# ChunLI-666/PointCloudProcessor

Hardware: AMD Instinct MI355X
Metric: Mpoints×frames/sec colorized (higher is better)
Workload: dtype f32/f64

## Files before the change

include/pcp_hip.h:

```cpp
#ifndef PCP_HIP_H
#define PCP_HIP_H

#include <stdint.h>

#ifdef __cplusplus
extern "C" {
#endif

#define PCP_ABI_VERSION 6

#define PCP_OK 0
#define PCP_ERR_INVALID (-1)
#define PCP_ERR_STATE (-2)
#define PCP_ERR_DEVICE (-3)
#define PCP_ERR_NOMEM (-4)
#define PCP_ERR_RANGE (-5)

typedef struct pcp_context pcp_context;

typedef struct pcp_pose {
  double x, y, z, qw, qx, qy, qz;
} pcp_pose;

typedef struct pcp_camera {
// ... 168 lines not shown
int pcp_nid_accumulate(pcp_context *ctx, const double T[16], int32_t bins);
int pcp_nid_histograms_device(pcp_context *ctx, void **device_ptr, int64_t *count);
int pcp_nid_finish(pcp_context *ctx, int32_t bins, double *cost, double grad6[6], int32_t *valid);
typedef int (*pcp_nid_eval_fn)(void *user, const double T[16], int32_t bins, double *cost, double grad6[6], int32_t *valid);
int pcp_nid_optimize_with(pcp_context *ctx, pcp_nid_eval_fn eval, void *user, const double T_init[16], int32_t bins,
                          int32_t max_outer_iterations, double T_out[16], double *final_cost, int32_t *evaluations);

int pcp_close_pairs(pcp_context *ctx, double radius, int64_t *points_with_close_neighbour);

int pcp_timing_enable(pcp_context *ctx, int32_t on);
int pcp_timing_reset(pcp_context *ctx);
int pcp_timing_get(pcp_context *ctx, int32_t kernel_id, double *total_ms, int64_t *launches);
const char *pcp_kernel_name(int32_t kernel_id);
int pcp_tile_mask_density(pcp_context *ctx, double *kept_fraction);
int pcp_tile_masks(pcp_context *ctx, int64_t *tiles, int32_t *mask_words, uint32_t *out_words);
int pcp_sor_redo_fraction(pcp_context *ctx, double *fraction);
int pcp_sor_distances(pcp_context *ctx, int64_t capacity, float *out_distance);
int pcp_selftest_arithmetic(pcp_context *ctx, int64_t samples, uint64_t seed, int64_t *mismatches_fp64,
                            int64_t *mismatches_fp32);

#ifdef __cplusplus
}
#endif
#endif
```

pointcloudprocessor_amd/capi.py:

```python
from __future__ import annotations

import ctypes as C
import os
import re

import numpy as np

from . import _build

PCP_OK = 0
PCP_ERR_INVALID = -1
PCP_ERR_STATE = -2
PCP_ERR_DEVICE = -3
PCP_ERR_NOMEM = -4
PCP_ERR_RANGE = -5

NID_EVAL_FN = C.CFUNCTYPE(C.c_int, C.c_void_p, C.POINTER(C.c_double), C.c_int32, C.POINTER(C.c_double), C.POINTER(C.c_double),
                          C.POINTER(C.c_int32))
K_PROJECT, K_DEPTH, K_COLOUR, K_VISIBILITY, K_MLS_GRID, K_MLS_FIT, K_MISC, K_SOR, K_MLS_VOXEL, K_TILE_MASK, K_NID, K_HPR = range(12)
K_COLOUR_SMOOTH = 12
K_COUNT = 13


class PcpError(RuntimeError):
# ... 627 lines not shown
        self._check(self.lib.pcp_tile_mask_density(self.h, C.byref(v)))
        return v.value

    def selftest_arithmetic(self, samples: int = 1 << 26, seed: int = 1):
        a, b = C.c_int64(), C.c_int64()
        self._check(self.lib.pcp_selftest_arithmetic(self.h, C.c_int64(samples), C.c_uint64(seed), C.byref(a), C.byref(b)))
        return a.value, b.value

    def tile_masks(self) -> np.ndarray:
        t, w = C.c_int64(), C.c_int32()
        self._check(self.lib.pcp_tile_masks(self.h, C.byref(t), C.byref(w), None))
        out = np.empty((t.value, w.value), np.uint32)
        self._check(self.lib.pcp_tile_masks(self.h, None, None, _ptr(out)))
        return out

    def kernel_name(self, kernel_id: int) -> str:
        return self.lib.pcp_kernel_name(C.c_int32(kernel_id)).decode()
```

pointcloudprocessor_amd/csrc/pcp_colour.hip:

```cpp
#include <algorithm>
#include <cfloat>
#include <cstdlib>

#include "pcp_device.hpp"
#include "pcp_hsv.hpp"
#include "pcp_scan.hpp"

namespace pcp {

constexpr int kBlock = 256;
constexpr uint32_t kFltMaxBits = 0x7f7fffffu;

template <bool kCommon>
__device__ __forceinline__ DevCamera common_camera(const DevCamera &in) {
  DevCamera c = in;
  if constexpr (kCommon) {
    c.cull_mode = PCP_CULL_ZBUFFER;
    c.enable_zbuf = 1;
    c.pretest = 1;
    c.ds_fast = 1;
  }
  return c;
}
inline bool is_common_camera(const DevCamera &c) {
// ... 127 lines not shown
  Interval rc = iv_add(iv_add(iv_scale(c.k1, r2), iv_scale(c.k2, r4)), iv_scale(c.k3, r6));
  rc.lo += 1.0;
  rc.hi += 1.0;
  const Interval t1 = iv_scale(2.0, iv_mul(xn, yn));
  const Interval t2 = iv_add(r2, iv_scale(2.0, x2));
  const Interval t3 = iv_add(r2, iv_scale(2.0, y2));
  const Interval xd = iv_pad(iv_add(iv_add(iv_mul(rc, xn), iv_scale(c.p1, t1)), iv_scale(c.p2, t2)));
  const Interval yd = iv_pad(iv_add(iv_add(iv_mul(rc, yn), iv_scale(c.p1, t3)), iv_scale(c.p2, t1)));
  Interval u = iv_pad(iv_scale(c.fx, xd)), v = iv_pad(iv_scale(c.fy, yd));
  u.lo += c.cx; u.hi += c.cx;
  v.lo += c.cy; v.hi += c.cy;
  if (!isfinite(u.lo + u.hi + v.lo + v.hi)) return 0;
  if (u.hi < static_cast<double>(c.u_lo) || u.lo > static_cast<double>(c.u_hi) ||
      v.hi < static_cast<double>(c.v_lo) || v.lo > static_cast<double>(c.v_hi))
    return 1;
  return (u.lo > static_cast<double>(c.u_lo) + 1.0 && u.hi < static_cast<double>(c.u_hi) - 1.0 &&
          v.lo > static_cast<double>(c.v_lo) + 1.0 && v.hi < static_cast<double>(c.v_hi) - 1.0)
             ? 2
             : 0;
}

constexpr int kTileGroup = 16;

__global__ __launch_bounds__(kBlock) void k_group_mask_flat(const float4 *__restrict__ spheres, int64_t groups, DevCamera cam,
                                                            const DevFrame *__restrict__ frames, int32_t n_frames,
                                                            int32_t w0, int32_t w1, int32_t words,
                                                            uint32_t *__restrict__ group_mask,
                                                            uint32_t *__restrict__ group_inside, int32_t cull_enabled,
                                                            int32_t *__restrict__ zeroed, int32_t n_zeroed,
                                                            unsigned long long *__restrict__ far_maps, int64_t far_cells) {
  const int64_t idx = static_cast<int64_t>(blockIdx.x) * kBlock + threadIdx.x;
  if (idx < n_zeroed) zeroed[idx] = 0;
// ... 157 lines not shown

__device__ __forceinline__ uint32_t range_bits(int32_t w, int32_t f0, int32_t f1) {
  const int32_t fb = max(f0, w << 5), fe = min(f1, (w << 5) + 32);
  const int32_t nb = fe - fb;
  return nb <= 0 ? 0u : (((nb >= 32) ? 0xffffffffu : ((1u << nb) - 1u)) << (fb & 31));
}

template <bool kCommon>
__global__ __launch_bounds__(kBlock) void k_depth_pass(const float *__restrict__ x, const float *__restrict__ y,
                                                       const float *__restrict__ z, int64_t n, DevCamera cam_in,
                                                       const DevFrame *__restrict__ frames, int32_t f0, int32_t f1,
                                                       unsigned long long *__restrict__ depth, int64_t cells,
                                                       int32_t depth_first_frame, uint32_t *__restrict__ tile_mask,
                                                       const uint32_t *__restrict__ tile_inside, int32_t words,
                                                       const int32_t *__restrict__ tile_order) {
  DevCamera cam = common_camera<kCommon>(cam_in);
  if constexpr (kCommon) cam.pretest = 0;
  __shared__ unsigned long long combine[kBlock];
  const int lane = threadIdx.x & 63;
  unsigned long long *tbl = combine + (threadIdx.x & ~63);
  const int64_t j = tile_order ? static_cast<int64_t>(tile_order[blockIdx.x]) * 64 + threadIdx.x
                               : static_cast<int64_t>(xcd_chunked_block()) * kBlock + threadIdx.x;
  const bool live = j < n;
  if (!__ballot(live)) return;
  const float px = live ? x[j] : 0.0f, py = live ? y[j] : 0.0f, pz = live ? z[j] : 0.0f;
  const int64_t tile = __builtin_amdgcn_readfirstlane(static_cast<int32_t>(j >> 6));
  const bool finite_sure = cam.frames_bounded != 0 && __all(fabsf(px) <= 0x1p40f && fabsf(py) <= 0x1p40f && fabsf(pz) <= 0x1p40f);
  unsigned long long *held_at = nullptr;
  unsigned long long held_bits = 0ull, held_seen = 0ull;
  auto settle_held = [&]() {
    if (held_at && held_bits < held_seen) atomicMin(held_at, held_bits);
    held_at = nullptr;
  };
  for (int32_t w = f0 >> 5; w <= (f1 - 1) >> 5; ++w) {
    const uint32_t in_range = range_bits(w, f0, f1);
    uint32_t todo = in_range;
    if (tile_mask) todo &= tile_mask[tile * words + w];
    todo = __builtin_amdgcn_readfirstlane(todo);
    const uint32_t inside = tile_inside ? __builtin_amdgcn_readfirstlane(tile_inside[tile * words + w]) : 0u;
    uint32_t seen = 0u;
    while (todo) {
      const int32_t b = __builtin_ctz(todo);
      const int32_t f = (w << 5) + b;
      todo &= todo - 1u;
      const DevFrame &fr = frames[f];
      const Projected p = project_point(cam, fr.w2c, px, py, pz, ((inside >> b) & 1u) == 0u, finite_sure);
      const bool in_map = live && p.cell >= 0;
      const bool cand = live && p.pixel >= 0 && (cam.enable_zbuf ? p.cell >= 0 : p.cell != -1);
      if (__ballot(cand)) seen |= 1u << b;
      settle_held();
      if (cam.enable_zbuf && __ballot(in_map)) {
        unsigned long long *map = depth + static_cast<uint64_t>(static_cast<uint32_t>(f - depth_first_frame)) * static_cast<uint32_t>(cells);
        unsigned long long key = ~0ull, sbits = 0ull;
        if (in_map) {
          sbits = static_cast<unsigned long long>(__double_as_longlong(sumsq64(p.xc, p.yc, p.zc)));
          key = (static_cast<unsigned long long>(static_cast<uint32_t>(p.cell)) << 32) | (sbits >> 32);
        }
        tbl[lane] = ~0ull;
        __builtin_amdgcn_wave_barrier();
        if (in_map) atomicMin(&tbl[p.cell & 63], key);
        __builtin_amdgcn_wave_barrier();
        if (in_map) {
          const unsigned long long got = tbl[p.cell & 63];
          if (got == key || static_cast<uint32_t>(got >> 32) != static_cast<uint32_t>(p.cell)) {
// ... 39 lines not shown
  float *score;
  uint32_t *rgb;
  int32_t *frame;
  int32_t *count;
};

struct MatchArgs {
  const uint8_t *in_a;
  unsigned long long *moved;
  float e2;
};

struct LabelOut {
  uint32_t *word;
};

template <bool kCommon, int kMatch, bool kOneShot, bool kLabel = false>
__global__ __launch_bounds__(kBlock) void k_colour_pass(const float *__restrict__ x, const float *__restrict__ y,
                                                        const float *__restrict__ z, int64_t n, DevCamera cam_in,
                                                        const DevFrame *__restrict__ frames, int32_t f0, int32_t f1,
                                                        const uint32_t *__restrict__ depth, int64_t cells,
                                                        const uint32_t *__restrict__ tile_mask, int32_t words,
                                                        const uint32_t *__restrict__ images, int64_t image_px,
                                                        TopState st, const int32_t *__restrict__ perm,
                                                        uint32_t *__restrict__ rgba, int32_t flags_in,
                                                        const uint32_t *__restrict__ hull_bits_in, MatchArgs mb,
                                                        [[maybe_unused]] LabelOut lab) {
  DevCamera cam = common_camera<kCommon>(cam_in);
  if constexpr (kMatch == 1) cam.match_mode = PCP_MATCH_IDENTITY;
  if constexpr (kMatch == 2 || kMatch == 3) cam.match_mode = PCP_MATCH_ROUNDTRIP;
  const uint32_t *__restrict__ hull_bits = kCommon ? nullptr : hull_bits_in;
  const int32_t flags = kOneShot ? 4 : flags_in;
  const int64_t j = static_cast<int64_t>(xcd_chunked_block()) * kBlock + threadIdx.x;
  const bool live = j < n;
  if (!__ballot(live)) return;
  const float px = live ? x[j] : 0.0f, py = live ? y[j] : 0.0f, pz = live ? z[j] : 0.0f;
  const int64_t tile = __builtin_amdgcn_readfirstlane(static_cast<int32_t>(j >> 6));
  const bool finite_sure = cam.frames_bounded != 0 && __all(fabsf(px) <= 0x1p40f && fabsf(py) <= 0x1p40f && fabsf(pz) <= 0x1p40f);
  Top5 t;
  t.init();
  if ((flags & 1) && live) {
    t.s0 = st.score[0 * n + j]; t.s1 = st.score[1 * n + j]; t.s2 = st.score[2 * n + j];
    t.s3 = st.score[3 * n + j]; t.s4 = st.score[4 * n + j];
    t.c0 = st.rgb[0 * n + j]; t.c1 = st.rgb[1 * n + j]; t.c2 = st.rgb[2 * n + j];
    t.c3 = st.rgb[3 * n + j]; t.c4 = st.rgb[4 * n + j];
    t.f0 = st.frame[0 * n + j]; t.f1 = st.frame[1 * n + j]; t.f2 = st.frame[2 * n + j];
    t.f3 = st.frame[3 * n + j]; t.f4 = st.frame[4 * n + j];
    t.count = st.count[j];
  }
  [[maybe_unused]] bool in_a = false;
  [[maybe_unused]] uint32_t moved = 0u;
  if constexpr (kMatch == 3) in_a = live && mb.in_a[j] != 0;
  for (int32_t w = f0 >> 5; w <= (f1 - 1) >> 5; ++w) {
    uint32_t todo = range_bits(w, f0, f1);
    if (tile_mask) todo &= tile_mask[tile * words + w];
    todo = __builtin_amdgcn_readfirstlane(todo);
    const uint32_t hull_word = (hull_bits && live) ? hull_bits[static_cast<int64_t>(w) * n + j] : 0xffffffffu;
    while (todo) {
      const int32_t f = (w << 5) + __builtin_ctz(todo);
      todo &= todo - 1u;
      const DevFrame &fr = frames[f];
      const Projected p = project_point<false>(cam, fr.w2c, px, py, pz, true, finite_sure);
      const bool cand = live && p.pixel >= 0 && (cam.enable_zbuf ? p.cell >= 0 : p.cell != -1) &&
                        ((hull_word >> (f & 31)) & 1u);
// ... 6 lines not shown
          if (keep) keep = roundtrip_sample_moved(cam, fr, px, py, pz, sx, sy, sz, mb.e2, moved) && !in_a;
        } else {
          if (cam.match_mode == PCP_MATCH_ROUNDTRIP && keep) keep = roundtrip_sample(cam, fr, px, py, pz, sx, sy, sz);
        }
        if (keep) {
          const uint32_t texel = images[static_cast<uint64_t>(static_cast<uint32_t>(f)) * static_cast<uint32_t>(image_px) + static_cast<uint32_t>(p.pixel)];
          t.insert(final_score(sx, sy, sz, fr.px, fr.py, fr.pz), kLabel ? texel : texel & 0xffffffu, f);
        }
      }
    }
  }
  if constexpr (kMatch == 3) {
    if (moved) atomicAdd(mb.moved, static_cast<unsigned long long>(moved));
  }
  if (!live) return;
  if (flags & 2) {
    st.score[0 * n + j] = t.s0; st.score[1 * n + j] = t.s1; st.score[2 * n + j] = t.s2;
    st.score[3 * n + j] = t.s3; st.score[4 * n + j] = t.s4;
    st.rgb[0 * n + j] = t.c0; st.rgb[1 * n + j] = t.c1; st.rgb[2 * n + j] = t.c2;
    st.rgb[3 * n + j] = t.c3; st.rgb[4 * n + j] = t.c4;
    st.frame[0 * n + j] = t.f0; st.frame[1 * n + j] = t.f1; st.frame[2 * n + j] = t.f2;
    st.frame[3 * n + j] = t.f3; st.frame[4 * n + j] = t.f4;
    st.count[j] = t.count;
  }
  if (flags & 4) {
    const int64_t o = perm[j];
    rgba[o] = t.finalise();
    if constexpr (kLabel) {
      uint32_t bad = 0u;
      lab.word[o] = t.labels(bad);
      if (bad) lab.word[n] = 1u;
    }
  }
}

__device__ __forceinline__ Top5 load_top5(const TopState &st, int64_t n, int64_t j) {
  Top5 t;
  t.s0 = st.score[0 * n + j]; t.s1 = st.score[1 * n + j]; t.s2 = st.score[2 * n + j];
  t.s3 = st.score[3 * n + j]; t.s4 = st.score[4 * n + j];
  t.c0 = st.rgb[0 * n + j]; t.c1 = st.rgb[1 * n + j]; t.c2 = st.rgb[2 * n + j];
  t.c3 = st.rgb[3 * n + j]; t.c4 = st.rgb[4 * n + j];
  t.f0 = st.frame[0 * n + j]; t.f1 = st.frame[1 * n + j]; t.f2 = st.frame[2 * n + j];
  t.f3 = st.frame[3 * n + j]; t.f4 = st.frame[4 * n + j];
  t.count = st.count[j];
  return t;
}
__global__ __launch_bounds__(kBlock) void k_finalise(int64_t n, TopState st, const int32_t *__restrict__ perm,
                                                     uint32_t *__restrict__ rgba) {
  const int64_t j = static_cast<int64_t>(blockIdx.x) * kBlock + threadIdx.x;
  if (j >= n) return;
  const Top5 t = load_top5(st, n, j);
  rgba[static_cast<int64_t>(perm[j])] = t.finalise();
}
__global__ __launch_bounds__(kBlock) void k_finalise_labels(int64_t n, TopState st, const int32_t *__restrict__ perm,
                                                            uint32_t *__restrict__ rgba, LabelOut lab) {
  const int64_t j = static_cast<int64_t>(blockIdx.x) * kBlock + threadIdx.x;
  if (j >= n) return;
  const Top5 t = load_top5(st, n, j);
  const int64_t o = perm[j];
  rgba[o] = t.finalise();
  uint32_t bad = 0u;
  lab.word[o] = t.labels(bad);
  if (bad) lab.word[n] = 1u;
}

template <bool kLabel>
__global__ __launch_bounds__(kBlock) void k_match_fixup(const float *__restrict__ x, const float *__restrict__ y,
                                                        const float *__restrict__ z, int64_t n, DevCamera cam,
                                                        const DevFrame *__restrict__ frames, int32_t f0, int32_t f1,
                                                        const uint32_t *__restrict__ depth, int64_t cells,
                                                        const uint32_t *__restrict__ tile_mask, int32_t words,
                                                        const uint32_t *__restrict__ images, int64_t image_px, TopState st,
                                                        const int32_t *__restrict__ perm, uint32_t *__restrict__ rgba,
                                                        int32_t flags, const uint32_t *__restrict__ hull_bits,
                                                        const int32_t *__restrict__ list, int64_t na,
                                                        const int64_t *__restrict__ off, const int32_t *__restrict__ cols,
                                                        [[maybe_unused]] LabelOut lab) {
  const int64_t a = static_cast<int64_t>(blockIdx.x) * kBlock + threadIdx.x;
// ... 55 lines not shown
}

template <bool kLabel>
inline auto colour_pass_kernel(bool common, int32_t match_mode, int32_t flags) {
  auto kernel = k_colour_pass<false, 0, false, kLabel>;
  if (common && match_mode == PCP_MATCH_IDENTITY)
    kernel = flags == 4 ? k_colour_pass<true, 1, true, kLabel> : k_colour_pass<true, 1, false, kLabel>;
  if (common && match_mode == PCP_MATCH_ROUNDTRIP)
    kernel = flags == 4 ? k_colour_pass<true, 2, true, kLabel> : k_colour_pass<true, 2, false, kLabel>;
  if (match_mode == PCP_MATCH_RADIUS)
    kernel = !common ? k_colour_pass<false, 3, false, kLabel>
                     : flags == 4 ? k_colour_pass<true, 3, true, kLabel> : k_colour_pass<true, 3, false, kLabel>;
  return kernel;
}

__device__ __forceinline__ uint64_t mix64(uint64_t v) {
  v += 0x9e3779b97f4a7c15ull;
  v = (v ^ (v >> 30)) * 0xbf58476d1ce4e5b9ull;
  v = (v ^ (v >> 27)) * 0x94d049bb133111ebull;
  return v ^ (v >> 31);
}
__device__ __forceinline__ bool same_f64(double a, double b) {
  if (a != a && b != b) return true;
  if (a == 0.0 && b == 0.0) return true;
  return __double_as_longlong(a) == __double_as_longlong(b);
}

__global__ __launch_bounds__(kBlock) void k_selftest_div64(int64_t samples, uint64_t seed,
                                                           unsigned long long *__restrict__ bad) {
  const int64_t i = static_cast<int64_t>(blockIdx.x) * kBlock + threadIdx.x;
// ... 328 lines not shown
                     ctx->mask_words, ctx->tile_work.p, ctx->work_hist.p);
  hipLaunchKernelGGL(k_work_scatter, dim3(sort_blocks), dim3(kBlock), 0, ctx->stream, ctx->tile_work.p, ctx->n_tiles,
                     ctx->work_hist.p, ctx->work_hist.p + kWorkBins, order);
  PCP_HIP_TRY(ctx, hipGetLastError());
  return PCP_OK;
}

static int ensure_hull_bits(pcp_context *ctx) {
  const size_t words = static_cast<size_t>((ctx->n_frames + 31) / 32);
  const size_t need = words * static_cast<size_t>(ctx->n) + 4;
  if (ctx->hull_bits.count < need || ctx->hull_valid.size() != static_cast<size_t>(ctx->n_frames)) {
    PCP_HIP_TRY(ctx, ctx->hull_bits.ensure(need));
    ctx->hull_valid.assign(static_cast<size_t>(ctx->n_frames), 0);
  }
  return PCP_OK;
}

static int ensure_depth(pcp_context *ctx) {
  const size_t need = static_cast<size_t>(cells_of(ctx)) * ctx->n_frames + 4;
  if (ctx->depth.count < need) {
    PCP_HIP_TRY(ctx, ctx->depth.ensure(need));
    std::fill(ctx->depth_valid.begin(), ctx->depth_valid.end(), uint8_t(0));
  }
  const int32_t words = (ctx->n_frames + 31) / 32;
  const size_t need_mask = static_cast<size_t>(words) * static_cast<size_t>(std::max<int64_t>(ctx->n_tiles, 1)) + 4;
  if (ctx->tile_mask.count < need_mask || ctx->mask_words != words) {
    PCP_HIP_TRY(ctx, ctx->tile_mask.ensure(need_mask));
    PCP_HIP_TRY(ctx, ctx->tile_inside.ensure(need_mask));
    PCP_HIP_TRY(ctx, ctx->tile_work.ensure(static_cast<size_t>(std::max<int64_t>(ctx->n_tiles, 1)) + 4));
    PCP_HIP_TRY(ctx, ctx->tile_order.ensure(static_cast<size_t>(std::max<int64_t>(ctx->n_tiles, 1)) + 4));
// ... 551 lines not shown
    return set_error(ctx, PCP_ERR_RANGE, "pcp_depth_pass: keyframe range [%d,%d) outside 0..%d", frame_begin, frame_end,
                     ctx->n_frames);
  if (frame_begin == frame_end) return PCP_OK;
  if ((rc = ensure_depth(ctx)) != PCP_OK) return rc;
  const int64_t cells = cells_of(ctx);
  const int64_t map_cells = static_cast<int64_t>(frame_end - frame_begin) * cells;
  const bool z_maps = ctx->n > 0 && ctx->dcam.enable_zbuf;
  if (z_maps) {
    PCP_HIP_TRY(ctx, ctx->depth_sq.ensure(static_cast<size_t>(map_cells) + 4));
  } else if ((rc = fill_u32(ctx, ctx->depth.p + static_cast<int64_t>(frame_begin) * cells, map_cells, kFltMaxBits)) != PCP_OK) {
    return rc;
  }
  if (ctx->n > 0) {
    const size_t plane = plane_of(ctx);
    const int32_t w0 = frame_begin >> 5, w1 = ((frame_end - 1) >> 5) + 1;
    static const bool cull_tiles = [] {
      const char *e = std::getenv("PCP_DISABLE_TILE_CULL");
      return !(e && e[0] == '1');
    }();
    {
      LaunchTimer t(ctx, PCP_K_TILE_MASK);
      const int64_t groups = div_up(ctx->n_tiles, kTileGroup);
      const float4 *tile_sph = reinterpret_cast<const float4 *>(ctx->tile_sphere.p);
      const size_t gwords = static_cast<size_t>(groups) * ctx->mask_words;
      PCP_HIP_TRY(ctx, ctx->group_mask.ensure(2 * gwords + 8));
      uint32_t *group_inside = ctx->group_mask.p + gwords + 4;
      hipLaunchKernelGGL(k_group_mask_flat, dim3(std::max(blocks_for(groups * (w1 - w0) * 32), blocks_for(2 * kWorkBins))),
                         dim3(kBlock), 0, ctx->stream, tile_sph + ctx->n_tiles, groups, ctx->dcam, ctx->frames.p, ctx->n_frames,
                         w0, w1, ctx->mask_words, ctx->group_mask.p, group_inside, cull_tiles ? 1 : 0, ctx->work_hist.p,
                         2 * kWorkBins, z_maps ? reinterpret_cast<unsigned long long *>(ctx->depth_sq.p) : nullptr,
                         z_maps ? map_cells : int64_t(0));
      hipLaunchKernelGGL(k_tile_mask_dense, dim3(static_cast<uint32_t>(div_up(groups * (w1 - w0), kBlock / 64))), dim3(kBlock),
                         0, ctx->stream, tile_sph, ctx->n_tiles, ctx->dcam, ctx->frames.p, ctx->n_frames, w0, w1,
                         ctx->mask_words, ctx->group_mask.p, group_inside, ctx->tile_mask.p, ctx->tile_inside.p, cull_tiles ? 1 : 0);
// ... 179 lines not shown
  if (one_shot)
    flags |= 4;
  else
    flags |= 2;
  MatchArgs mb{nullptr, nullptr, 0.0f};
  if (radius) {
    mb = MatchArgs{ctx->match_in_a.p, ctx->match_moved.p, ctx->match_e2};
    PCP_HIP_TRY(ctx, hipMemsetAsync(ctx->match_moved.p, 0, 8, ctx->stream));
  }
  const uint32_t *hull = ctx->cull.cull_mode == PCP_CULL_HPR ? ctx->hull_bits.p : static_cast<const uint32_t *>(nullptr);
  {
    LaunchTimer t(ctx, PCP_K_COLOUR);
    const bool common = is_common_camera(ctx->dcam) && ctx->cull.cull_mode != PCP_CULL_HPR;
    const bool label = ctx->label_fusion;
    const LabelOut lab{label ? ctx->labels.p : nullptr};
    auto kernel = label ? colour_pass_kernel<true>(common, ctx->dcam.match_mode, flags)
                        : colour_pass_kernel<false>(common, ctx->dcam.match_mode, flags);
    hipLaunchKernelGGL(kernel, dim3(blocks_for(ctx->n)), dim3(kBlock), 0, ctx->stream, ctx->sxyz.p, ctx->sxyz.p + plane,
                       ctx->sxyz.p + 2 * plane, ctx->n, ctx->dcam, ctx->frames.p, frame_begin, frame_end, ctx->depth.p,
                       cells_of(ctx), ctx->tile_mask.p, ctx->mask_words, ctx->images.p,
                       static_cast<int64_t>(ctx->dcam.img_w) * ctx->dcam.img_h, st, ctx->perm.p, result, flags, hull, mb, lab);
    PCP_HIP_TRY(ctx, hipGetLastError());
    if (radius && ctx->match_a > 0) {
      hipLaunchKernelGGL(label ? k_match_fixup<true> : k_match_fixup<false>, dim3(blocks_for(ctx->match_a)), dim3(kBlock), 0, ctx->stream, ctx->sxyz.p,
                         ctx->sxyz.p + plane, ctx->sxyz.p + 2 * plane, ctx->n, ctx->dcam, ctx->frames.p, frame_begin, frame_end,
                         ctx->depth.p, cells_of(ctx), ctx->tile_mask.p, ctx->mask_words, ctx->images.p,
                         static_cast<int64_t>(ctx->dcam.img_w) * ctx->dcam.img_h, st, ctx->perm.p, result, flags, hull,
                         ctx->match_list.p, ctx->match_a, ctx->match_off.p, ctx->match_cols.p, lab);
      PCP_HIP_TRY(ctx, hipGetLastError());
    }
  }
  if (!one_shot) ctx->colour_state_live = true;
  if (radius) {
    unsigned long long moved = 0;
    unsigned long long *dst = ctx->readback ? static_cast<unsigned long long *>(ctx->readback) : &moved;
    PCP_HIP_TRY(ctx, hipMemcpyAsync(dst, ctx->match_moved.p, 8, hipMemcpyDeviceToHost, ctx->stream));
// ... 178 lines not shown

int pcp_tile_masks(pcp_context *ctx, int64_t *tiles, int32_t *mask_words, uint32_t *out_words) {
  if (!ctx) return PCP_ERR_INVALID;
  if (!ctx->tile_mask.p || ctx->n_tiles == 0 || ctx->n_frames == 0)
    return set_error(ctx, PCP_ERR_STATE, "pcp_tile_masks: no masks (call pcp_depth_pass)");
  if (tiles) *tiles = ctx->n_tiles;
  if (mask_words) *mask_words = ctx->mask_words;
  if (out_words) {
    PCP_HIP_TRY(ctx, hipMemcpyAsync(out_words, ctx->tile_mask.p, static_cast<size_t>(ctx->n_tiles) * ctx->mask_words * 4,
                                    hipMemcpyDeviceToHost, ctx->stream));
    PCP_HIP_TRY(ctx, hipStreamSynchronize(ctx->stream));
  }
  return PCP_OK;
}

int pcp_colour_result_device(pcp_context *ctx, void **device_ptr, int64_t *n_words) {
  if (!ctx) return PCP_ERR_INVALID;
  if (!ctx->colour_result_live)
    return set_error(ctx, PCP_ERR_STATE, "pcp_colour_result_device: no result (call pcp_colorize / pcp_colour_finalise)");
  if (device_ptr) *device_ptr = ctx->rgba2[ctx->rgba_cur].p;
  if (n_words) *n_words = ctx->n;
  return PCP_OK;
}

int pcp_set_label_fusion(pcp_context *ctx, int32_t enable) {
  if (!ctx) return PCP_ERR_INVALID;
  const bool on = enable != 0;
  if (on != ctx->label_fusion && ctx->colour_state_live)
    return set_error(ctx, PCP_ERR_STATE, "pcp_set_label_fusion: a top-5 accumulation is live (its lists %s the masks): "
                     "call pcp_colour_reset first", ctx->label_fusion ? "hold" : "do not hold");
// ... 58 lines not shown
```

pointcloudprocessor_amd/csrc/pcp_context.hip:

```cpp
#include <algorithm>
#include <cfloat>
#include <cmath>
#include <cstdlib>
#include <new>
#include <vector>

#include "pcp_internal.hpp"
#include "pcp_scan.hpp"

namespace pcp {

static thread_local std::string g_error;

int set_error(const pcp_context *ctx, int code, const char *fmt, ...) {
  char buf[1024];
  va_list ap;
  va_start(ap, fmt);
  vsnprintf(buf, sizeof(buf), fmt, ap);
  va_end(ap);
  if (ctx)
    ctx->error = buf;
  else
    g_error = buf;
  return code;
// ... 314 lines not shown
        lo[a] = fmin(lo[a], red[a][k]);
        hi[a] = fmax(hi[a], red[3 + a][k]);
      }
    __syncthreads();
  }
  float c[3];
#pragma unroll
  for (int a = 0; a < 3; ++a) c[a] = static_cast<float>(0.5 * (lo[a] + hi[a]));
  double r2 = 0.0;
#pragma unroll
  for (int q = 0; q < kPer; ++q)
    if (have[q]) {
      const double dx = static_cast<double>(px[q]) - static_cast<double>(c[0]);
      const double dy = static_cast<double>(py[q]) - static_cast<double>(c[1]);
      const double dz = static_cast<double>(pz[q]) - static_cast<double>(c[2]);
      r2 = fmax(r2, (dx * dx + dy * dy) + dz * dz);
    }
  for (int o = (kLanes < 64 ? kLanes : 64) / 2; o >= 1; o >>= 1) r2 = fmax(r2, __shfl_xor(r2, o, 64));
  if (kLanes > 64) {
    if ((threadIdx.x & 63) == 0) red[6][threadIdx.x >> 6] = r2;
    __syncthreads();
    for (int k = 0; k < kUpBlock / 64; ++k) r2 = fmax(r2, red[6][k]);
  }
  if (l == 0 && sphere < count) {
    float r = static_cast<float>(sqrt(r2) * (1.0 + 1e-6));
    r = isfinite(r) ? __uint_as_float(__float_as_uint(r) + 1u) : r;
    out[sphere] = make_float4(c[0], c[1], c[2], r);
  }
}

static inline uint32_t up_blocks(int64_t n) { return static_cast<uint32_t>(std::max<int64_t>(1, (n + kUpBlock - 1) / kUpBlock)); }
// ... 449 lines not shown
  d.qk2 = static_cast<float>(cam->k2);
  d.qk3 = static_cast<float>(cam->k3);
  d.qp1 = static_cast<float>(cam->p1);
  d.qp2 = static_cast<float>(cam->p2);
  {
    const float ds = static_cast<float>(cp.downsample_factor);
    const bool hpr = cp.cull_mode != PCP_CULL_ZBUFFER;
    const float cw = hpr ? static_cast<float>(d.cull_w) : ds * static_cast<float>(d.enable_zbuf ? d.mw : d.cull_w);
    const float ch = hpr ? static_cast<float>(d.cull_h) : ds * static_cast<float>(d.enable_zbuf ? d.mh : d.cull_h);
    d.u_lo = -(ds + 0.5f);
    d.v_lo = -(ds + 0.5f);
    d.u_hi = std::max(cw, static_cast<float>(d.img_w)) + 0.5f;
    d.v_hi = std::max(ch, static_cast<float>(d.img_h)) + 0.5f;
  }
  if (const char *e = std::getenv("PCP_DISABLE_PRETEST")) d.pretest = (e[0] == '1') ? 0 : 1;

  ctx->have_camera = true;
  for (hipStream_t us : ctx->upload_stream)
    if (us) (void)hipStreamSynchronize(us);
  std::fill(ctx->image_pending.begin(), ctx->image_pending.end(), uint8_t(0));
  ctx->image_set.assign(ctx->image_set.size(), 0);
  ctx->mask_set.assign(ctx->mask_set.size(), 0);
  std::fill(ctx->depth_valid.begin(), ctx->depth_valid.end(), uint8_t(0));
  ctx->hull_valid.clear();
  ctx->colour_state_live = false;
  ctx->colour_result_live = false;
  ctx->labels_live = false;
  return PCP_OK;
}

int pcp_upload_cloud(pcp_context *ctx, const float *x, const float *y, const float *z, int64_t n) {
// ... 129 lines not shown
```

pointcloudprocessor_amd/csrc/pcp_device.hpp:

```cpp
#pragma once

#include <hip/hip_runtime.h>

#include <cfloat>
#include <cstdint>

#include "pcp_internal.hpp"

namespace pcp {

__device__ __forceinline__ void xform(const float *__restrict__ m, float x, float y, float z, float &xc, float &yc,
                                      float &zc) {
  xc = x * m[0] + (y * m[1] + (z * m[2] + m[3]));
  yc = x * m[4] + (y * m[5] + (z * m[6] + m[7]));
  zc = x * m[8] + (y * m[9] + (z * m[10] + m[11]));
}

__device__ __forceinline__ void divide_xy_by_z(float xc, float yc, float zc, double &xn, double &yn, bool finite_sure = false) {
  const double X = xc, Y = yc, Z = zc;
  if (finite_sure || (xc - xc) + (yc - yc) + (zc - zc) == 0.0f) {
    double r = __builtin_amdgcn_rcp(Z);
    double e = __builtin_fma(-Z, r, 1.0);
    r = __builtin_fma(r, e, r);
    e = __builtin_fma(-Z, r, 1.0);
// ... 52 lines not shown

template <bool kShortDiv = true>
__device__ __forceinline__ int32_t cull_cell(const DevCamera &c, double u, double v) {
  if (c.cull_mode == PCP_CULL_HPR_CANDIDATES) {
    return (u > -1.0 && u < c.cull_wd && v > -1.0 && v < c.cull_hd) ? -2 : -1;
  }
  const float cxf = kShortDiv ? div_by_ds(c, static_cast<float>(u)) : static_cast<float>(u) / c.ds_f;
  const float cyf = kShortDiv ? div_by_ds(c, static_cast<float>(v)) : static_cast<float>(v) / c.ds_f;
  const int32_t cx = cell_of_quotient(cxf, c.cull_wf), cy = cell_of_quotient(cyf, c.cull_hf);
  if ((cx < 0) | (cy < 0)) return -1;
  return ((cx < c.mw) & (cy < c.mh)) ? cy * c.mw + cx : (c.enable_zbuf ? -1 : -2);
}

__device__ __forceinline__ int32_t colour_pixel(const DevCamera &c, double u, double v) {
  if (!(u > -1.0 && u < c.img_wd && v > -1.0 && v < c.img_hd)) return -1;
  return static_cast<int32_t>(v) * c.img_w + static_cast<int32_t>(u);
}

__device__ __forceinline__ double range64(float xc, float yc, float zc) {
  const double X = xc, Y = yc, Z = zc;
  return sqrt((X * X + Y * Y) + Z * Z);
}

__device__ __forceinline__ bool surely_rejected(const DevCamera &c, float xc, float yc, float zc) {
  const float rz = __builtin_amdgcn_rcpf(zc);
  const float xn = xc * rz, yn = yc * rz;
  const float x2 = xn * xn, y2 = yn * yn;
  const float r2 = x2 + y2, r4 = r2 * r2, r6 = r2 * r4;
  const float rc = __builtin_fmaf(c.qk3, r6, __builtin_fmaf(c.qk2, r4, __builtin_fmaf(c.qk1, r2, 1.0f)));
  const float ra = __builtin_fmaf(fabsf(c.qk3), r6, __builtin_fmaf(fabsf(c.qk2), r4, __builtin_fmaf(fabsf(c.qk1), r2, 1.0f)));
// ... 195 lines not shown
```

pointcloudprocessor_amd/csrc/pcp_internal.hpp:

```cpp
#pragma once

#include <hip/hip_runtime.h>

#include <cstdarg>
#include <cstdint>
#include <chrono>
#include <cstdio>
#include <cstring>
#include <string>
#include <vector>

#include "pcp_hip.h"

namespace pcp {

struct DevCamera {
  double fx, fy, cx, cy;
  double k1, k2, p1, p2, k3;
  double slack;
  float ds_f;
  double img_wd, img_hd;
  float cull_wf, cull_hf;
  float ds_rcp;
  int32_t ds_fast;
  int32_t ds;
  int32_t img_w, img_h;
  int32_t cull_w, cull_h;
  int32_t mw, mh;
  int32_t enable_zbuf;
  int32_t cull_mode;
  int32_t match_mode;
  double cull_wd, cull_hd;
  float match_r2;
  int32_t pretest;
  int32_t frames_bounded;
  float qfx, qfy, qcx, qcy;
  float qk1, qk2, qk3, qp1, qp2;
  float u_lo, u_hi, v_lo, v_hi;
};

struct DevFrame {
  float w2c[12];
  float c2w[12];
  double px, py, pz;
  double norm_bound;
  float c2w_inv[12];
  float pad_[4];
};
static_assert(sizeof(DevFrame) == 192, "DevFrame layout");

constexpr int kTopM = 5;

struct TimingSlot {
// ... 333 lines not shown
```

Baseline: 1.847 million.

## Skip per-point visibility tests for tiles proven fully inside frame

Adds a specialised colour-pass kernel for the common z-buffer camera that uses per-tile 'sure inside' bits to skip the per-point bounds and cell checks, and uses the same sure bits in the depth pass. The sure-inside test is tightened to the intersection of the depth-map and image extents so skipped checks stay valid. NaN handling in the bound-radius reduction is made conservative. A probe API and script report the share of sure tiles. The cost targeted is the redundant per-point projection bounds checking and branching in the hot colour and depth loops.

```diff
diff --git a/include/pcp_hip.h b/include/pcp_hip.h
--- a/include/pcp_hip.h
+++ b/include/pcp_hip.h
@@ -206,6 +206,7 @@
 const char *pcp_kernel_name(int32_t kernel_id);
 int pcp_tile_mask_density(pcp_context *ctx, double *kept_fraction);
 int pcp_tile_masks(pcp_context *ctx, int64_t *tiles, int32_t *mask_words, uint32_t *out_words);
+int pcp_tile_sure_flags(pcp_context *ctx, int32_t frame, uint8_t *out_flags);
 int pcp_sor_redo_fraction(pcp_context *ctx, double *fraction);
 int pcp_sor_distances(pcp_context *ctx, int64_t capacity, float *out_distance);
 int pcp_selftest_arithmetic(pcp_context *ctx, int64_t samples, uint64_t seed, int64_t *mismatches_fp64,
diff --git a/pointcloudprocessor_amd/capi.py b/pointcloudprocessor_amd/capi.py
--- a/pointcloudprocessor_amd/capi.py
+++ b/pointcloudprocessor_amd/capi.py
@@ -665,5 +665,10 @@
         self._check(self.lib.pcp_tile_masks(self.h, None, None, _ptr(out)))
         return out
 
+    def tile_sure_flags(self, frame: int) -> np.ndarray:
+        out = np.zeros(self.n, np.uint8)
+        self._check(self.lib.pcp_tile_sure_flags(self.h, C.c_int32(frame), _ptr(out)))
+        return out
+
     def kernel_name(self, kernel_id: int) -> str:
         return self.lib.pcp_kernel_name(C.c_int32(kernel_id)).decode()
diff --git a/pointcloudprocessor_amd/csrc/pcp_colour.hip b/pointcloudprocessor_amd/csrc/pcp_colour.hip
--- a/pointcloudprocessor_amd/csrc/pcp_colour.hip
+++ b/pointcloudprocessor_amd/csrc/pcp_colour.hip
@@ -165,8 +165,8 @@
   if (u.hi < static_cast<double>(c.u_lo) || u.lo > static_cast<double>(c.u_hi) ||
       v.hi < static_cast<double>(c.v_lo) || v.lo > static_cast<double>(c.v_hi))
     return 1;
-  return (u.lo > static_cast<double>(c.u_lo) + 1.0 && u.hi < static_cast<double>(c.u_hi) - 1.0 &&
-          v.lo > static_cast<double>(c.v_lo) + 1.0 && v.hi < static_cast<double>(c.v_hi) - 1.0)
+  return (u.lo > static_cast<double>(c.su_lo) + 1.0 && u.hi < static_cast<double>(c.su_hi) - 1.0 &&
+          v.lo > static_cast<double>(c.sv_lo) + 1.0 && v.hi < static_cast<double>(c.sv_hi) - 1.0)
              ? 2
              : 0;
 }
@@ -354,8 +354,7 @@
                                                        int32_t depth_first_frame, uint32_t *__restrict__ tile_mask,
                                                        const uint32_t *__restrict__ tile_inside, int32_t words,
                                                        const int32_t *__restrict__ tile_order) {
-  DevCamera cam = common_camera<kCommon>(cam_in);
-  if constexpr (kCommon) cam.pretest = 0;
+  const DevCamera cam = common_camera<kCommon>(cam_in);
   __shared__ unsigned long long combine[kBlock];
   const int lane = threadIdx.x & 63;
   unsigned long long *tbl = combine + (threadIdx.x & ~63);
@@ -377,17 +376,36 @@
     uint32_t todo = in_range;
     if (tile_mask) todo &= tile_mask[tile * words + w];
     todo = __builtin_amdgcn_readfirstlane(todo);
-    const uint32_t inside = tile_inside ? __builtin_amdgcn_readfirstlane(tile_inside[tile * words + w]) : 0u;
+    const uint32_t sure_word = tile_inside ? __builtin_amdgcn_readfirstlane(tile_inside[tile * words + w]) : 0u;
     uint32_t seen = 0u;
     while (todo) {
       const int32_t b = __builtin_ctz(todo);
       const int32_t f = (w << 5) + b;
       todo &= todo - 1u;
       const DevFrame &fr = frames[f];
-      const Projected p = project_point(cam, fr.w2c, px, py, pz, ((inside >> b) & 1u) == 0u, finite_sure);
-      const bool in_map = live && p.cell >= 0;
-      const bool cand = live && p.pixel >= 0 && (cam.enable_zbuf ? p.cell >= 0 : p.cell != -1);
-      if (__ballot(cand)) seen |= 1u << b;
+      const bool sure = ((sure_word >> b) & 1u) != 0u;
+      Projected p;
+      bool in_map;
+      if constexpr (kCommon) {
+        xform(fr.w2c, px, py, pz, p.xc, p.yc, p.zc);
+        double u, v;
+        project_uv(cam, p.xc, p.yc, p.zc, u, v, finite_sure);
+        float qx, qy;
+        common_cell_quotients(cam, u, v, qx, qy);
+        in_map = live;
+        if (sure) {
+          seen |= 1u << b;
+        } else {
+          in_map = live && p.zc > 0.0f && common_cell_ok(cam, qx, qy);
+          if (__ballot(in_map && colour_pixel_ok(cam, u, v))) seen |= 1u << b;
+        }
+        p.cell = common_cell_index(cam, qx, qy);
+      } else {
+        p = project_point(cam, fr.w2c, px, py, pz, !sure, finite_sure);
+        in_map = live && p.cell >= 0;
+        const bool cand = live && p.pixel >= 0 && (cam.enable_zbuf ? p.cell >= 0 : p.cell != -1);
+        if (__ballot(cand)) seen |= 1u << b;
+      }
       settle_held();
       if (cam.enable_zbuf && __ballot(in_map)) {
         unsigned long long *map = depth + static_cast<uint64_t>(static_cast<uint32_t>(f - depth_first_frame)) * static_cast<uint32_t>(cells);
@@ -457,6 +475,42 @@
 struct LabelOut {
   uint32_t *word;
 };
+
+__device__ __forceinline__ Top5 load_top5(const TopState &st, int64_t n, int64_t j) {
+  Top5 t;
+  t.s0 = st.score[0 * n + j]; t.s1 = st.score[1 * n + j]; t.s2 = st.score[2 * n + j];
+  t.s3 = st.score[3 * n + j]; t.s4 = st.score[4 * n + j];
+  t.c0 = st.rgb[0 * n + j]; t.c1 = st.rgb[1 * n + j]; t.c2 = st.rgb[2 * n + j];
+  t.c3 = st.rgb[3 * n + j]; t.c4 = st.rgb[4 * n + j];
+  t.f0 = st.frame[0 * n + j]; t.f1 = st.frame[1 * n + j]; t.f2 = st.frame[2 * n + j];
+  t.f3 = st.frame[3 * n + j]; t.f4 = st.frame[4 * n + j];
+  t.count = st.count[j];
+  return t;
+}
+__device__ __forceinline__ void store_top5(const TopState &st, int64_t n, int64_t j, const Top5 &t) {
+  st.score[0 * n + j] = t.s0; st.score[1 * n + j] = t.s1; st.score[2 * n + j] = t.s2;
+  st.score[3 * n + j] = t.s3; st.score[4 * n + j] = t.s4;
+  st.rgb[0 * n + j] = t.c0; st.rgb[1 * n + j] = t.c1; st.rgb[2 * n + j] = t.c2;
+  st.rgb[3 * n + j] = t.c3; st.rgb[4 * n + j] = t.c4;
+  st.frame[0 * n + j] = t.f0; st.frame[1 * n + j] = t.f1; st.frame[2 * n + j] = t.f2;
+  st.frame[3 * n + j] = t.f3; st.frame[4 * n + j] = t.f4;
+  st.count[j] = t.count;
+}
+template <bool kLabel>
+__device__ __forceinline__ void colour_finish(int32_t flags, const TopState &st, int64_t n, int64_t j, const Top5 &t,
+                                              const int32_t *__restrict__ perm, uint32_t *__restrict__ rgba,
+                                              [[maybe_unused]] const LabelOut &lab) {
+  if (flags & 2) store_top5(st, n, j, t);
+  if (flags & 4) {
+    const int64_t o = perm[j];
+    rgba[o] = t.finalise();
+    if constexpr (kLabel) {
+      uint32_t bad = 0u;
+      lab.word[o] = t.labels(bad);
+      if (bad) lab.word[n] = 1u;
+    }
+  }
+}
 
 template <bool kCommon, int kMatch, bool kOneShot, bool kLabel = false>
 __global__ __launch_bounds__(kBlock) void k_colour_pass(const float *__restrict__ x, const float *__restrict__ y,
@@ -482,15 +536,7 @@
   const bool finite_sure = cam.frames_bounded != 0 && __all(fabsf(px) <= 0x1p40f && fabsf(py) <= 0x1p40f && fabsf(pz) <= 0x1p40f);
   Top5 t;
   t.init();
-  if ((flags & 1) && live) {
-    t.s0 = st.score[0 * n + j]; t.s1 = st.score[1 * n + j]; t.s2 = st.score[2 * n + j];
-    t.s3 = st.score[3 * n + j]; t.s4 = st.score[4 * n + j];
-    t.c0 = st.rgb[0 * n + j]; t.c1 = st.rgb[1 * n + j]; t.c2 = st.rgb[2 * n + j];
-    t.c3 = st.rgb[3 * n + j]; t.c4 = st.rgb[4 * n + j];
-    t.f0 = st.frame[0 * n + j]; t.f1 = st.frame[1 * n + j]; t.f2 = st.frame[2 * n + j];
-    t.f3 = st.frame[3 * n + j]; t.f4 = st.frame[4 * n + j];
-    t.count = st.count[j];
-  }
+  if ((flags & 1) && live) t = load_top5(st, n, j);
   [[maybe_unused]] bool in_a = false;
   [[maybe_unused]] uint32_t moved = 0u;
   if constexpr (kMatch == 3) in_a = live && mb.in_a[j] != 0;
@@ -527,37 +573,9 @@
     if (moved) atomicAdd(mb.moved, static_cast<unsigned long long>(moved));
   }
   if (!live) return;
-  if (flags & 2) {
-    st.score[0 * n + j] = t.s0; st.score[1 * n + j] = t.s1; st.score[2 * n + j] = t.s2;
-    st.score[3 * n + j] = t.s3; st.score[4 * n + j] = t.s4;
-    st.rgb[0 * n + j] = t.c0; st.rgb[1 * n + j] = t.c1; st.rgb[2 * n + j] = t.c2;
-    st.rgb[3 * n + j] = t.c3; st.rgb[4 * n + j] = t.c4;
-    st.frame[0 * n + j] = t.f0; st.frame[1 * n + j] = t.f1; st.frame[2 * n + j] = t.f2;
-    st.frame[3 * n + j] = t.f3; st.frame[4 * n + j] = t.f4;
-    st.count[j] = t.count;
-  }
-  if (flags & 4) {
-    const int64_t o = perm[j];
-    rgba[o] = t.finalise();
-    if constexpr (kLabel) {
-      uint32_t bad = 0u;
-      lab.word[o] = t.labels(bad);
-      if (bad) lab.word[n] = 1u;
-    }
-  }
-}
-
-__device__ __forceinline__ Top5 load_top5(const TopState &st, int64_t n, int64_t j) {
-  Top5 t;
-  t.s0 = st.score[0 * n + j]; t.s1 = st.score[1 * n + j]; t.s2 = st.score[2 * n + j];
-  t.s3 = st.score[3 * n + j]; t.s4 = st.score[4 * n + j];
-  t.c0 = st.rgb[0 * n + j]; t.c1 = st.rgb[1 * n + j]; t.c2 = st.rgb[2 * n + j];
-  t.c3 = st.rgb[3 * n + j]; t.c4 = st.rgb[4 * n + j];
-  t.f0 = st.frame[0 * n + j]; t.f1 = st.frame[1 * n + j]; t.f2 = st.frame[2 * n + j];
-  t.f3 = st.frame[3 * n + j]; t.f4 = st.frame[4 * n + j];
-  t.count = st.count[j];
-  return t;
-}
+  colour_finish<kLabel>(flags, st, n, j, t, perm, rgba, lab);
+}
+
 __global__ __launch_bounds__(kBlock) void k_finalise(int64_t n, TopState st, const int32_t *__restrict__ perm,
                                                      uint32_t *__restrict__ rgba) {
   const int64_t j = static_cast<int64_t>(blockIdx.x) * kBlock + threadIdx.x;
@@ -575,6 +593,77 @@
   uint32_t bad = 0u;
   lab.word[o] = t.labels(bad);
   if (bad) lab.word[n] = 1u;
+}
+
+struct SureVisits {};
+template <typename Form, int kMatch, bool kOneShot, bool kLabel>
+__global__ __launch_bounds__(kBlock) void k_colour_pass(const float *__restrict__ x, const float *__restrict__ y,
+                                                        const float *__restrict__ z, int64_t n, DevCamera cam_in,
+                                                        const DevFrame *__restrict__ frames, int32_t f0, int32_t f1,
+                                                        const uint32_t *__restrict__ depth, int64_t cells,
+                                                        const uint32_t *__restrict__ tile_mask,
+                                                        const uint32_t *__restrict__ tile_sure, int32_t words,
+                                                        uint32_t image_px, const uint32_t *__restrict__ images,
+                                                        TopState st, const int32_t *__restrict__ perm,
+                                                        uint32_t *__restrict__ rgba, int32_t flags_in,
+                                                        MatchArgs mb,
+                                                        [[maybe_unused]] LabelOut lab) {
+  DevCamera cam = common_camera<true>(cam_in);
+  if constexpr (kMatch == 1) cam.match_mode = PCP_MATCH_IDENTITY;
+  if constexpr (kMatch == 2 || kMatch == 3) cam.match_mode = PCP_MATCH_ROUNDTRIP;
+  const int32_t flags = kOneShot ? 4 : flags_in;
+  const int64_t j = static_cast<int64_t>(xcd_chunked_block()) * kBlock + threadIdx.x;
+  const bool live = j < n;
+  if (!__ballot(live)) return;
+  const float px = live ? x[j] : 0.0f, py = live ? y[j] : 0.0f, pz = live ? z[j] : 0.0f;
+  const int64_t tile = __builtin_amdgcn_readfirstlane(static_cast<int32_t>(j >> 6));
+  const bool finite_sure = cam.frames_bounded != 0 && __all(fabsf(px) <= 0x1p40f && fabsf(py) <= 0x1p40f && fabsf(pz) <= 0x1p40f);
+  Top5 t;
+  t.init();
+  if ((flags & 1) && live) t = load_top5(st, n, j);
+  [[maybe_unused]] bool in_a = false;
+  [[maybe_unused]] uint32_t moved = 0u;
+  if constexpr (kMatch == 3) in_a = live && mb.in_a[j] != 0;
+  for (int32_t w = f0 >> 5; w <= (f1 - 1) >> 5; ++w) {
+    uint32_t todo = range_bits(w, f0, f1) & tile_mask[tile * words + w];
+    todo = __builtin_amdgcn_readfirstlane(todo);
+    const uint32_t sure_word = __builtin_amdgcn_readfirstlane(tile_sure[tile * words + w]);
+    while (todo) {
+      const int32_t b = __builtin_ctz(todo);
+      const int32_t f = (w << 5) + b;
+      todo &= todo - 1u;
+      const DevFrame &fr = frames[f];
+      Projected p;
+      xform(fr.w2c, px, py, pz, p.xc, p.yc, p.zc);
+      double u, v;
+      project_uv(cam, p.xc, p.yc, p.zc, u, v, finite_sure);
+      float qx, qy;
+      common_cell_quotients(cam, u, v, qx, qy);
+      bool cand = live;
+      if (!((sure_word >> b) & 1u)) cand = live && p.zc > 0.0f && common_cell_ok(cam, qx, qy) && colour_pixel_ok(cam, u, v);
+      p.cell = common_cell_index(cam, qx, qy);
+      p.pixel = colour_pixel_index(cam, u, v);
+      if (cand) {
+        const uint32_t dbits = depth[static_cast<uint64_t>(static_cast<uint32_t>(f)) * static_cast<uint32_t>(cells) + static_cast<uint32_t>(p.cell)];
+        bool keep = keep_by_depth(p.xc, p.yc, p.zc, static_cast<double>(__uint_as_float(dbits)) + cam.slack);
+        float sx = p.xc, sy = p.yc, sz = p.zc;
+        if constexpr (kMatch == 3) {
+          if (keep) keep = roundtrip_sample_moved(cam, fr, px, py, pz, sx, sy, sz, mb.e2, moved) && !in_a;
+        } else {
+          if (cam.match_mode == PCP_MATCH_ROUNDTRIP && keep) keep = roundtrip_sample(cam, fr, px, py, pz, sx, sy, sz);
+        }
+        if (keep) {
+          const uint32_t texel = images[static_cast<uint64_t>(static_cast<uint32_t>(f)) * image_px + static_cast<uint32_t>(p.pixel)];
+          t.insert(final_score(sx, sy, sz, fr.px, fr.py, fr.pz), kLabel ? texel : texel & 0xffffffu, f);
+        }
+      }
+    }
+  }
+  if constexpr (kMatch == 3) {
+    if (moved) atomicAdd(mb.moved, static_cast<unsigned long long>(moved));
+  }
+  if (!live) return;
+  colour_finish<kLabel>(flags, st, n, j, t, perm, rgba, lab);
 }
 
 template <bool kLabel>
@@ -660,6 +749,16 @@
   return kernel;
 }
 
+template <bool kLabel>
+inline auto sure_pass_kernel(int32_t match_mode, int32_t flags) {
+  auto kernel = flags == 4 ? k_colour_pass<SureVisits, 1, true, kLabel> : k_colour_pass<SureVisits, 1, false, kLabel>;
+  if (match_mode == PCP_MATCH_ROUNDTRIP)
+    kernel = flags == 4 ? k_colour_pass<SureVisits, 2, true, kLabel> : k_colour_pass<SureVisits, 2, false, kLabel>;
+  if (match_mode == PCP_MATCH_RADIUS)
+    kernel = flags == 4 ? k_colour_pass<SureVisits, 3, true, kLabel> : k_colour_pass<SureVisits, 3, false, kLabel>;
+  return kernel;
+}
+
 __device__ __forceinline__ uint64_t mix64(uint64_t v) {
   v += 0x9e3779b97f4a7c15ull;
   v = (v ^ (v >> 30)) * 0xbf58476d1ce4e5b9ull;
@@ -1018,6 +1117,14 @@
     ctx->hull_valid.assign(static_cast<size_t>(ctx->n_frames), 0);
   }
   return PCP_OK;
+}
+
+static bool tile_cull_enabled() {
+  static const bool on = [] {
+    const char *e = std::getenv("PCP_DISABLE_TILE_CULL");
+    return !(e && e[0] == '1');
+  }();
+  return on;
 }
 
 static int ensure_depth(pcp_context *ctx) {
@@ -1599,10 +1706,7 @@
   if (ctx->n > 0) {
     const size_t plane = plane_of(ctx);
     const int32_t w0 = frame_begin >> 5, w1 = ((frame_end - 1) >> 5) + 1;
-    static const bool cull_tiles = [] {
-      const char *e = std::getenv("PCP_DISABLE_TILE_CULL");
-      return !(e && e[0] == '1');
-    }();
+    const bool cull_tiles = tile_cull_enabled();
     {
       LaunchTimer t(ctx, PCP_K_TILE_MASK);
       const int64_t groups = div_up(ctx->n_tiles, kTileGroup);
@@ -1812,12 +1916,21 @@
     const bool common = is_common_camera(ctx->dcam) && ctx->cull.cull_mode != PCP_CULL_HPR;
     const bool label = ctx->label_fusion;
     const LabelOut lab{label ? ctx->labels.p : nullptr};
-    auto kernel = label ? colour_pass_kernel<true>(common, ctx->dcam.match_mode, flags)
-                        : colour_pass_kernel<false>(common, ctx->dcam.match_mode, flags);
-    hipLaunchKernelGGL(kernel, dim3(blocks_for(ctx->n)), dim3(kBlock), 0, ctx->stream, ctx->sxyz.p, ctx->sxyz.p + plane,
-                       ctx->sxyz.p + 2 * plane, ctx->n, ctx->dcam, ctx->frames.p, frame_begin, frame_end, ctx->depth.p,
-                       cells_of(ctx), ctx->tile_mask.p, ctx->mask_words, ctx->images.p,
-                       static_cast<int64_t>(ctx->dcam.img_w) * ctx->dcam.img_h, st, ctx->perm.p, result, flags, hull, mb, lab);
+    if (common && tile_cull_enabled()) {
+      auto kernel = label ? sure_pass_kernel<true>(ctx->dcam.match_mode, flags) : sure_pass_kernel<false>(ctx->dcam.match_mode, flags);
+      hipLaunchKernelGGL(kernel, dim3(blocks_for(ctx->n)), dim3(kBlock), 0, ctx->stream, ctx->sxyz.p, ctx->sxyz.p + plane,
+                         ctx->sxyz.p + 2 * plane, ctx->n, ctx->dcam, ctx->frames.p, frame_begin, frame_end, ctx->depth.p,
+                         cells_of(ctx), ctx->tile_mask.p, ctx->tile_inside.p, ctx->mask_words,
+                         static_cast<uint32_t>(ctx->dcam.img_w) * static_cast<uint32_t>(ctx->dcam.img_h), ctx->images.p, st,
+                         ctx->perm.p, result, flags, mb, lab);
+    } else {
+      auto kernel = label ? colour_pass_kernel<true>(common, ctx->dcam.match_mode, flags)
+                          : colour_pass_kernel<false>(common, ctx->dcam.match_mode, flags);
+      hipLaunchKernelGGL(kernel, dim3(blocks_for(ctx->n)), dim3(kBlock), 0, ctx->stream, ctx->sxyz.p, ctx->sxyz.p + plane,
+                         ctx->sxyz.p + 2 * plane, ctx->n, ctx->dcam, ctx->frames.p, frame_begin, frame_end, ctx->depth.p,
+                         cells_of(ctx), ctx->tile_mask.p, ctx->mask_words, ctx->images.p,
+                         static_cast<int64_t>(ctx->dcam.img_w) * ctx->dcam.img_h, st, ctx->perm.p, result, flags, hull, mb, lab);
+    }
     PCP_HIP_TRY(ctx, hipGetLastError());
     if (radius && ctx->match_a > 0) {
       hipLaunchKernelGGL(label ? k_match_fixup<true> : k_match_fixup<false>, dim3(blocks_for(ctx->match_a)), dim3(kBlock), 0, ctx->stream, ctx->sxyz.p,
@@ -2026,6 +2139,28 @@
   return PCP_OK;
 }
 
+int pcp_tile_sure_flags(pcp_context *ctx, int32_t frame, uint8_t *out_flags) {
+  if (!ctx) return PCP_ERR_INVALID;
+  if (!ctx->tile_mask.p || !ctx->tile_inside.p || ctx->n_tiles == 0 || ctx->n_frames == 0)
+    return set_error(ctx, PCP_ERR_STATE, "pcp_tile_sure_flags: no masks (call pcp_depth_pass)");
+  if (frame < 0 || frame >= ctx->n_frames)
+    return set_error(ctx, PCP_ERR_RANGE, "pcp_tile_sure_flags: keyframe %d outside 0..%d", frame, ctx->n_frames);
+  if (static_cast<size_t>(frame) >= ctx->depth_valid.size() || !ctx->depth_valid[static_cast<size_t>(frame)])
+    return set_error(ctx, PCP_ERR_STATE, "pcp_tile_sure_flags: pcp_depth_pass has not covered keyframe %d", frame);
+  if (!out_flags) return set_error(ctx, PCP_ERR_INVALID, "pcp_tile_sure_flags: NULL output");
+  PCP_HIP_TRY(ctx, hipSetDevice(ctx->device));
+  std::vector<uint32_t> sure(static_cast<size_t>(ctx->n_tiles) * ctx->mask_words);
+  std::vector<int32_t> perm(static_cast<size_t>(ctx->n));
+  PCP_HIP_TRY(ctx, hipMemcpyAsync(sure.data(), ctx->tile_inside.p, sure.size() * 4, hipMemcpyDeviceToHost, ctx->stream));
+  PCP_HIP_TRY(ctx, hipMemcpyAsync(perm.data(), ctx->perm.p, perm.size() * 4, hipMemcpyDeviceToHost, ctx->stream));
+  PCP_HIP_TRY(ctx, hipStreamSynchronize(ctx->stream));
+  for (int64_t j = 0; j < ctx->n; ++j) {
+    const uint32_t word = sure[static_cast<size_t>(j >> 6) * ctx->mask_words + (frame >> 5)];
+    out_flags[perm[static_cast<size_t>(j)]] = static_cast<uint8_t>((word >> (frame & 31)) & 1u);
+  }
+  return PCP_OK;
+}
+
 int pcp_colour_result_device(pcp_context *ctx, void **device_ptr, int64_t *n_words) {
   if (!ctx) return PCP_ERR_INVALID;
   if (!ctx->colour_result_live)
diff --git a/pointcloudprocessor_amd/csrc/pcp_context.hip b/pointcloudprocessor_amd/csrc/pcp_context.hip
--- a/pointcloudprocessor_amd/csrc/pcp_context.hip
+++ b/pointcloudprocessor_amd/csrc/pcp_context.hip
@@ -352,7 +352,8 @@
       const double dx = static_cast<double>(px[q]) - static_cast<double>(c[0]);
       const double dy = static_cast<double>(py[q]) - static_cast<double>(c[1]);
       const double dz = static_cast<double>(pz[q]) - static_cast<double>(c[2]);
-      r2 = fmax(r2, (dx * dx + dy * dy) + dz * dz);
+      const double d2 = (dx * dx + dy * dy) + dz * dz;
+      r2 = d2 == d2 ? fmax(r2, d2) : HUGE_VAL;
     }
   for (int o = (kLanes < 64 ? kLanes : 64) / 2; o >= 1; o >>= 1) r2 = fmax(r2, __shfl_xor(r2, o, 64));
   if (kLanes > 64) {
@@ -832,7 +833,12 @@
     d.v_hi = std::max(ch, static_cast<float>(d.img_h)) + 0.5f;
   }
   if (const char *e = std::getenv("PCP_DISABLE_PRETEST")) d.pretest = (e[0] == '1') ? 0 : 1;
-
+  {
+    const bool common = cp.cull_mode == PCP_CULL_ZBUFFER && d.enable_zbuf == 1 && d.pretest == 1 && d.ds_fast == 1;
+    d.su_lo = d.sv_lo = common ? -1.0f : 0.0f;
+    d.su_hi = common ? static_cast<float>(std::min(cp.downsample_factor * d.mw, d.img_w)) : 0.0f;
+    d.sv_hi = common ? static_cast<float>(std::min(cp.downsample_factor * d.mh, d.img_h)) : 0.0f;
+  }
   ctx->have_camera = true;
   for (hipStream_t us : ctx->upload_stream)
     if (us) (void)hipStreamSynchronize(us);
diff --git a/pointcloudprocessor_amd/csrc/pcp_device.hpp b/pointcloudprocessor_amd/csrc/pcp_device.hpp
--- a/pointcloudprocessor_amd/csrc/pcp_device.hpp
+++ b/pointcloudprocessor_amd/csrc/pcp_device.hpp
@@ -90,6 +90,23 @@
 
 __device__ __forceinline__ int32_t colour_pixel(const DevCamera &c, double u, double v) {
   if (!(u > -1.0 && u < c.img_wd && v > -1.0 && v < c.img_hd)) return -1;
+  return static_cast<int32_t>(v) * c.img_w + static_cast<int32_t>(u);
+}
+
+__device__ __forceinline__ bool colour_pixel_ok(const DevCamera &c, double u, double v) {
+  return u > -1.0 && u < c.img_wd && v > -1.0 && v < c.img_hd;
+}
+__device__ __forceinline__ void common_cell_quotients(const DevCamera &c, double u, double v, float &qx, float &qy) {
+  qx = div_by_ds(c, static_cast<float>(u));
+  qy = div_by_ds(c, static_cast<float>(v));
+}
+__device__ __forceinline__ bool common_cell_ok(const DevCamera &c, float qx, float qy) {
+  return fminf(qx, qy) > -1.0f && qx < static_cast<float>(c.mw) && qy < static_cast<float>(c.mh);
+}
+__device__ __forceinline__ int32_t common_cell_index(const DevCamera &c, float qx, float qy) {
+  return static_cast<int32_t>(qy) * c.mw + static_cast<int32_t>(qx);
+}
+__device__ __forceinline__ int32_t colour_pixel_index(const DevCamera &c, double u, double v) {
   return static_cast<int32_t>(v) * c.img_w + static_cast<int32_t>(u);
 }
 
diff --git a/pointcloudprocessor_amd/csrc/pcp_internal.hpp b/pointcloudprocessor_amd/csrc/pcp_internal.hpp
--- a/pointcloudprocessor_amd/csrc/pcp_internal.hpp
+++ b/pointcloudprocessor_amd/csrc/pcp_internal.hpp
@@ -37,6 +37,7 @@
   float qfx, qfy, qcx, qcy;
   float qk1, qk2, qk3, qp1, qp2;
   float u_lo, u_hi, v_lo, v_hi;
+  float su_lo, su_hi, sv_lo, sv_hi;
 };
 
 struct DevFrame {
diff --git a/profiles/sure_share_probe.py b/profiles/sure_share_probe.py
--- /dev/null
+++ b/profiles/sure_share_probe.py
@@ -0,0 +1,29 @@
+#!/usr/bin/env python3
+import json
+import os
+import sys
+
+import numpy as np
+
+sys.path.insert(0, os.path.dirname(os.path.dirname(os.path.abspath(__file__))))
+import torch
+
+from pointcloudprocessor_amd import capi, synth
+
+N = int(sys.argv[1]) if len(sys.argv) > 1 else 10_000_000
+F = int(sys.argv[2]) if len(sys.argv) > 2 else 256
+x, y, z, _ = synth.make_cloud(N)
+poses, _ = synth.make_trajectory(F)
+ctx = capi.Context(0)
+ctx.set_camera(capi.camera_from_dict(synth.camera_dict("cfg")))
+ctx.upload_cloud(x, y, z)
+ctx.set_frames(poses)
+ctx.depth_pass()
+masks = ctx.tile_masks()
+tiles = masks.shape[0]
+colour_visits = int(np.unpackbits(masks.view(np.uint8)).sum())
+sure_points = sum(int(ctx.tile_sure_flags(f).sum(dtype=np.int64)) for f in range(F))
+res = {"points": N, "keyframes": F, "tiles": int(tiles), "pairs": int(tiles) * F, "colour_pass_visits": colour_visits,
+       "sure_point_frames": sure_points, "sure_pairs_approx": round(sure_points / 64.0, 1),
+       "sure_share_of_colour_visits": round(sure_points / 64.0 / max(colour_visits, 1), 4)}
+print(json.dumps(res))
```

Result: faster. 1.892 million (median of 6 runs) (+2.4%).
